# IONIQ6000/av1-go

Hardware: AMD Instinct MI355X
Metric: encoded 4K30 frames/sec (whole node) at fixed QP; PSNR-Y delta vs libaom (higher is better)
Workload: dtype u16

## Files before the change

### av1-go_amd/csrc/av1_entropy_kernels.hip

```cpp
#include <string.h>
#include <vector>
#include "av1_ops_cdfs.hpp"
#include "av1_ops8.hpp"
#include "av1mi_internal.hpp"

namespace av1mi {
using namespace av1ops;

struct Av1EntLaunch {
  FrameView fv;
  int nframes, sbr_n, sbc_n;
  BlockInfo *info;
  op_t *ops; uint32_t ops_cap;
  uint32_t *grouped; uint32_t grouped_cap;
  uint16_t *slot_total, *slot_base;
  uint16_t *rec;
  uint32_t *nops;
  uint8_t *slots; uint32_t slot_cap;
  uint32_t *tile_size;
  uint64_t *tile_off;
  uint32_t *status;
  uint8_t *out; uint64_t out_cap;
  const uint16_t *cdf_image; int cdf_words;
  SlotTable tab;
// ... 4 lines not shown

template <int kKey = -1> __device__ __forceinline__ FrameView frame_view(const Av1EntLaunch &L, int f) {
  FrameView v = L.fv;
  const long nb = (long)v.w8 * v.h8;
  if (kKey < 0 ? v.key != 0 : kKey != 0) { v.y_mode += nb * f; v.uv_mode += nb * f; }
  else { v.mv += nb * 2 * f; v.skip += nb * f; }
  v.lev_y += nb * 64 * f; v.lev_u += nb * 16 * f; v.lev_v += nb * 16 * f;
  v.info = L.info + nb * f;
  if (L.lr_on_frame) for (int p = 0; p < 3; p++) v.lr_on[p] = v.lr_on[p] && L.lr_on_frame[f * 3 + p];
  return v;
}

__global__ __launch_bounds__(256) void k_av1_info(Av1EntLaunch L) {
  const long nb = (long)L.fv.w8 * L.fv.h8, i = (long)blockIdx.x * 256 + threadIdx.x;
  if (i >= nb * L.nframes) return;
  const int f = (int)(i / nb), b = (int)(i - (long)f * nb);
  const FrameView v = frame_view<0>(L, f);
  BlockInfo o = {};
  inter_mode_decision(v, b / v.w8, b % v.w8, &o);
  L.info[nb * f + b] = o;
}

struct TileWave {
  template <class T> using Var = LaneVar<T, 1>;
  template <class F> __device__ __forceinline__ void each(F f) { f((int)threadIdx.x); __syncthreads(); }
  __device__ __forceinline__ int scan(Var<int> &v) {
    const int lane = (int)threadIdx.x, x = v.v[0];
    int inc = x;
#pragma unroll
    for (int d = 1; d < 64; d <<= 1) {
      const int y = __shfl_up(inc, d, 64);
      if (lane >= d) inc += y;
    }
    v.v[0] = inc - x;
    return __shfl(inc, 63, 64);
  }
  __device__ __forceinline__ int first(Var<int> &v) { return __shfl(v.v[0], 0, 64); }
};

__global__ __launch_bounds__(64) __attribute__((amdgpu_waves_per_eu(2, 8))) void k_av1_tokens(Av1EntLaunch L) {
  const int tiles = L.sbr_n * L.sbc_n, t = blockIdx.x, f = t / tiles, tt = t - f * tiles, sbr = tt / L.sbc_n, sbc = tt - sbr * L.sbc_n;
  if (sbr < L.sb_rows32) return;
  const FrameView v = frame_view(L, f);
  __shared__ Tile8Mem S;
  const int below = tiles - L.sb_rows32 * L.sbc_n;
  uint16_t *rec = L.rec + ((size_t)f * below + (tt - (tiles - below))) * kBlocksPerTile * kBlockRecords;
  TileWave w;
  const int n = tok_tile8(w, S, v, sbr, sbc, rec, L.ops + (size_t)t * L.ops_cap, L.ops_cap, L.grouped + (size_t)t * L.grouped_cap,
                          L.slot_total + (size_t)t * S_MAX, L.slot_base + (size_t)t * S_MAX);
  if (threadIdx.x == 0) {
    if (n < 0) atomicOr(L.status, 1u);
    L.nops[t] = n < 0 ? 0u : (uint32_t)n;
  }
}

__global__ __launch_bounds__(64) void k_av1_tokens32(Av1EntLaunch L) {
  __shared__ Tile32Mem S;
  const int tiles = L.sbr_n * L.sbc_n, band = L.sb_rows32 * L.sbc_n, f = blockIdx.x / band, tt = blockIdx.x - f * band, sbr = tt / L.sbc_n, sbc = tt - sbr * L.sbc_n;
  const size_t t = (size_t)f * tiles + tt;
  const FrameView v = frame_view<1>(L, f);
  TileWave w;
  const int n = tok_tile32(w, S, v, sbr, sbc, L.ops + t * L.ops_cap, L.ops_cap, L.grouped + t * L.grouped_cap, L.slot_total + t * S_MAX, L.slot_base + t * S_MAX);
  if (threadIdx.x == 0) {
    if (n < 0) atomicOr(L.status, 1u);
    L.nops[t] = n < 0 ? 0u : (uint32_t)n;
  }
}

__global__ __launch_bounds__(64) void k_av1_chains(Av1EntLaunch L, int ntiles_all, int ngroups) {
  const int xcd = blockIdx.x & 7, j = blockIdx.x >> 3, nslots = L.nslots;
  const int g = (j / nslots) * 8 + xcd, sl = j - (j / nslots) * nslots, lane = threadIdx.x, t = g * 64 + lane;
  if (g >= ngroups) return;
  __shared__ __attribute__((aligned(16))) uint16_t s_big[64 * 16];
  const int n = L.tab.nsym[sl], off = L.tab.off[sl];
  int cnt = 0, base = 0;
  bool mine = t < ntiles_all;
  if (mine && L.band) { const int tiles = L.sbr_n * L.sbc_n, sbr = (t % tiles) / L.sbc_n; mine = (sbr < L.sb_rows32) == (L.band == 1); }
  if (mine) { cnt = L.slot_total[(size_t)t * S_MAX + sl]; base = L.slot_base[(size_t)t * S_MAX + sl]; }
  if (!__any(cnt > 0)) return;
  const size_t tt = t < ntiles_all ? (size_t)t : 0;
  op_t *list = L.ops + tt * L.ops_cap;
  const uint32_t *grouped = L.grouped + tt * L.grouped_cap + base;
  if (n <= 4) {
    const uint32_t *iw = reinterpret_cast<const uint32_t *>(L.cdf_image) + (off >> 1);
    uint64_t cdf = (uint64_t)iw[0] | ((uint64_t)iw[1] << 32);
    const uint4 *g4 = reinterpret_cast<const uint4 *>(grouped);
    const uint4 z = make_uint4(0, 0, 0, 0);
    uint4 c0 = cnt > 0 ? g4[0] : z, c1 = cnt > 4 ? g4[1] : z, c2 = cnt > 8 ? g4[2] : z, c3 = cnt > 12 ? g4[3] : z;
    auto four = [&](const uint4 &v, int e) {
      if (e < cnt) list[v.x >> 4] = small_step(cdf, (int)(v.x & 15), n);
      if (e + 1 < cnt) list[v.y >> 4] = small_step(cdf, (int)(v.y & 15), n);
      if (e + 2 < cnt) list[v.z >> 4] = small_step(cdf, (int)(v.z & 15), n);
      if (e + 3 < cnt) list[v.w >> 4] = small_step(cdf, (int)(v.w & 15), n);
    };
#pragma unroll 1
    for (int e = 0; e < cnt; e += 16) {
      const uint4 *nx = g4 + (e >> 2) + 4;
      const uint4 n0 = e + 16 < cnt ? nx[0] : z, n1 = e + 20 < cnt ? nx[1] : z, n2 = e + 24 < cnt ? nx[2] : z, n3 = e + 28 < cnt ? nx[3] : z;
      four(c0, e); four(c1, e + 4); four(c2, e + 8); four(c3, e + 12);
      c0 = n0; c1 = n1; c2 = n2; c3 = n3;
    }
  } else {
    uint16_t *cdf = s_big + lane * 16;
    {
      const uint4 *iw = reinterpret_cast<const uint4 *>(L.cdf_image + off);
      uint4 *d = reinterpret_cast<uint4 *>(cdf);
      d[0] = iw[0];
      d[1] = n > 8 ? iw[1] : make_uint4(0, 0, 0, 0);
    }
#pragma unroll 1
    for (int e = 0; e < cnt; e++) {
      const uint32_t v = grouped[e];
      const int s = (int)(v & 15);
      list[v >> 4] = s >= kSplitHorz ? split_tuple(cdf, s) : big_step(cdf, s, n);
    }
  }
}

constexpr int kRingOps = 64, kLaneWords = kRingOps * 2 + Coder::kStage + 8;

__global__ __launch_bounds__(64) void k_av1_code(Av1EntLaunch L, int ntiles_all) {
  __shared__ __attribute__((aligned(16))) uint16_t s_lane[64 * kLaneWords];
  const int lane = threadIdx.x, t = blockIdx.x * 64 + lane;
  const bool live = t < ntiles_all;
  uint32_t *ring = reinterpret_cast<uint32_t *>(s_lane + lane * kLaneWords);
  Coder c;
  c.init(L.slots + (size_t)(live ? t : 0) * L.slot_cap, (int)L.slot_cap, s_lane + lane * kLaneWords + kRingOps * 2);
  const int n = live ? (int)L.nops[t] : 0;
  const uint4 *ops4 = reinterpret_cast<const uint4 *>(L.ops + (size_t)(live ? t : 0) * L.ops_cap);
  uint4 r0, r1, r2, r3, r4, r5, r6, r7;
  r0 = r1 = r2 = r3 = r4 = r5 = r6 = r7 = make_uint4(0, 0, 0, 0);
  int w = 0;
  bool pend = false;
  auto request = [&]() {
    const uint4 *p = ops4 + (w >> 2);
    if (w < n) r0 = p[0];
    if (w + 4 < n) r1 = p[1];
    if (w + 8 < n) r2 = p[2];
    if (w + 12 < n) r3 = p[3];
    if (w + 16 < n) r4 = p[4];
    if (w + 20 < n) r5 = p[5];
    if (w + 24 < n) r6 = p[6];
    if (w + 28 < n) r7 = p[7];
    pend = w < n;
  };
  auto take = [&]() {
    uint4 *q = reinterpret_cast<uint4 *>(ring + (w & 32));
    q[0] = r0; q[1] = r1; q[2] = r2; q[3] = r3; q[4] = r4; q[5] = r5; q[6] = r6; q[7] = r7;
    w += 32;
  };
  request();
  if (pend) { take(); request(); }
  int i = 0, lit_left = 0;
  uint32_t op = ring[0], op_next = ring[1], op_next2 = ring[2];
  for (;;) {
    if (!__any(lit_left > 0 || i < n)) break;
    if (__any((pend && w - i < 24) || c.ns >= Coder::kStage - 8)) {
      if (pend && w - i <= 32) { take(); request(); }
      c.spill();
    }
#pragma unroll
    for (int q = 0; q < 8; q++) {
      if (lit_left > 0 || i < n) {
        const uint32_t fetched = ring[(i + 3) & (kRingOps - 1)];
        uint32_t tup = op;
        if (lit_left == 0 && (op >> 31)) lit_left = (int)((op >> 27) & 15);
        if (lit_left > 0) {
          lit_left--;
          tup = (op >> lit_left) & 1 ? (1u << 19) | (256u << 9) : (2u << 19) | (512u << 9) | 256u;
        }
        c.encode_tuple(tup);
        if (lit_left == 0) { i++; op = op_next; op_next = op_next2; op_next2 = fetched; }
      }
    }
  }
  if (!live) return;
  int sz = n ? c.finish() : -1;
  if (sz < 0) { if (n) atomicOr(L.status, 2u); sz = 0; }
  L.tile_size[t] = (uint32_t)sz;
}

__global__ __launch_bounds__(1024) void k_av1_scan(Av1EntLaunch L, int ntiles_all) {
  __shared__ uint64_t part[1024];
  const int tid = threadIdx.x, per = (ntiles_all + 1023) / 1024, i0 = tid * per, i1 = min(i0 + per, ntiles_all);
  uint64_t s = 0;
  for (int i = i0; i < i1; i++) s += L.tile_size[i];
  part[tid] = s;
  __syncthreads();
  for (int d = 1; d < 1024; d <<= 1) {
    const uint64_t y = tid >= d ? part[tid - d] : 0;
    __syncthreads();
    part[tid] += y;
    __syncthreads();
  }
  uint64_t run = part[tid] - s;
  for (int i = i0; i < i1; i++) { L.tile_off[i] = run; run += L.tile_size[i]; }
  if (tid == 1023) {
    L.tile_off[ntiles_all] = part[1023];
    if (part[1023] > L.out_cap) atomicOr(L.status, 4u);
  }
}
__global__ __launch_bounds__(64) void k_av1_gather(Av1EntLaunch L) {
  const int t = blockIdx.x;
  const uint32_t n = L.tile_size[t];
  const uint64_t off = L.tile_off[t];
  if (off + n > L.out_cap) return;
  const uint8_t *src = L.slots + (size_t)t * L.slot_cap;
  uint8_t *dst = L.out + off;
  const uint32_t head = min(n, (uint32_t)((16 - (reinterpret_cast<uintptr_t>(dst) & 15)) & 15)), body = (n - head) >> 4, tail0 = head + (body << 4);
  if (threadIdx.x < head) dst[threadIdx.x] = src[threadIdx.x];
  for (uint32_t i = threadIdx.x; i < body; i += 64) {
    uint4 v;
    __builtin_memcpy(&v, src + head + 16 * i, 16);
    *reinterpret_cast<uint4 *>(dst + head + 16 * i) = v;
  }
  if (tail0 + threadIdx.x < n) dst[tail0 + threadIdx.x] = src[tail0 + threadIdx.x];
}

hipError_t launch_av1_front(av1mi_ctx *ctx, const Av1EntLaunch &L, hipStream_t s) {
  const long nb = (long)L.fv.w8 * L.fv.h8 * L.nframes;
  const int ntiles_all = L.sbr_n * L.sbc_n * L.nframes, ngroups = (ntiles_all + 63) / 64;
  ProfToken t = ctx_prof_begin(ctx, AV1MI_K_ENTROPY_TOKENS, s);
  if (!L.fv.key) hipLaunchKernelGGL(k_av1_info, dim3((unsigned)((nb + 255) / 256)), dim3(256), 0, s, L);
  if (L.sb_rows32 < L.sbr_n) hipLaunchKernelGGL(k_av1_tokens, dim3((unsigned)ntiles_all), dim3(64), 0, s, L);
  if (L.sb_rows32) hipLaunchKernelGGL(k_av1_tokens32, dim3((unsigned)(L.sb_rows32 * L.sbc_n * L.nframes)), dim3(64), 0, s, L);
  ctx_prof_end(ctx, t, s);
  t = ctx_prof_begin(ctx, AV1MI_K_ENTROPY_CHAINS, s);
  Av1EntLaunch C = L;
  C.nslots = L.fv.key ? S_KEY_END : S_INTER_END; C.band = L.sb_rows32 ? 2 : 0;
  if (L.sb_rows32 < L.sbr_n) hipLaunchKernelGGL(k_av1_chains, dim3((unsigned)(((ngroups + 7) / 8) * 8 * C.nslots)), dim3(64), 0, s, C, ntiles_all, ngroups);
  if (L.sb_rows32) {
    C.nslots = K_END; C.band = 1; C.tab = L.tab32; C.cdf_image = L.cdf_image32;
    hipLaunchKernelGGL(k_av1_chains, dim3((unsigned)(((ngroups + 7) / 8) * 8 * C.nslots)), dim3(64), 0, s, C, ntiles_all, ngroups);
  }
  ctx_prof_end(ctx, t, s);
  return hipGetLastError();
}
hipError_t launch_av1_back(av1mi_ctx *ctx, const Av1EntLaunch &L, hipStream_t s) {
  const int ntiles_all = L.sbr_n * L.sbc_n * L.nframes;
  ProfToken t = ctx_prof_begin(ctx, AV1MI_K_ENTROPY, s);
  hipLaunchKernelGGL(k_av1_code, dim3((unsigned)((ntiles_all + 63) / 64)), dim3(64), 0, s, L, ntiles_all);
  ctx_prof_end(ctx, t, s);
  t = ctx_prof_begin(ctx, AV1MI_K_ENTROPY_PACK, s);
  hipLaunchKernelGGL(k_av1_scan, dim3(1), dim3(1024), 0, s, L, ntiles_all);
  hipLaunchKernelGGL(k_av1_gather, dim3((unsigned)ntiles_all), dim3(64), 0, s, L);
  ctx_prof_end(ctx, t, s);
  return hipGetLastError();
}

}

struct av1mi_av1ent_state {
  void *info = nullptr, *ops[2] = { nullptr, nullptr }, *nops[2] = { nullptr, nullptr }, *grouped = nullptr, *slot_tb = nullptr, *rec = nullptr, *slots = nullptr, *tile_off = nullptr, *status = nullptr;
  size_t info_b = 0, ops_b[2] = { 0, 0 }, nops_b[2] = { 0, 0 }, grouped_b = 0, slot_tb_b = 0, rec_b = 0, slots_b = 0, off_b = 0;
  hipEvent_t lists_ready[2] = { nullptr, nullptr }, lists_free[2] = { nullptr, nullptr };
  bool free_recorded[2] = { false, false };
  unsigned long jobs = 0;
  av1mi::Av1EntLaunch pending[2];
  uint64_t *pending_total[2] = { nullptr, nullptr };
  bool pending_valid[2] = { false, false };
  size_t last_tiles = 0;
  uint16_t *d_image[2][4] = {};
  uint16_t *d_image32[4] = {};
  av1ops::SlotTable tab32;
  int image_words[2] = { 0, 0 };
  av1ops::SlotTable tab[2];
};

namespace {
int grow(av1mi_ctx *ctx, void **p, size_t *have, size_t need) {
  if (*have >= need) return AV1MI_OK;
  if (*p) (void)hipFree(*p);
  *p = nullptr; *have = 0;
  if (hipMalloc(p, need) != hipSuccess) return av1mi::ctx_fail(ctx, AV1MI_E_NOMEM, "AV1 entropy scratch: hipMalloc(%zu) failed", need);
  *have = need;
  return AV1MI_OK;
}
}

extern "C" {

uint32_t av1mi_av1_entropy_ops_per_tile(void) { return 32768; }
uint32_t av1mi_av1_entropy_slot_bytes(void) { return 16384; }

}

int av1mi::av1_entropy_front(av1mi_ctx *ctx, const av1mi_av1_entropy_job *j, hipStream_t front, int *ticket) {
  if (!ctx || !ticket) return AV1MI_E_INVAL;
  *ticket = -1;
  if (!j) return av1mi::ctx_fail(ctx, AV1MI_E_INVAL, "null job");
  if (hipSetDevice(av1mi::ctx_device(ctx)) != hipSuccess) return av1mi::ctx_fail(ctx, AV1MI_E_DEVICE, "hipSetDevice failed");
  if (j->width <= 0 || j->height <= 0 || (j->width & 7) || (j->height & 7) || j->width > 4096 || j->height > 4096)
    return av1mi::ctx_fail(ctx, AV1MI_E_INVAL, "frame %dx%d must be a multiple of 8, at most 4096x4096", j->width, j->height);
  if (j->nframes < 0 || j->nframes > 4096 || j->base_q_idx < 1 || j->base_q_idx > 255) return av1mi::ctx_fail(ctx, AV1MI_E_INVAL, "bad nframes / base_q_idx");
  const void *need[] = { j->d_lev_y, j->d_lev_u, j->d_lev_v, j->d_out, j->d_tile_size, j->d_total, j->key ? (const void *)j->d_modes_y : (const void *)j->d_mvs,
                         j->key ? (const void *)j->d_modes_uv : (const void *)j->d_skip };
  for (const void *p : need) if (!p) return av1mi::ctx_fail(ctx, AV1MI_E_INVAL, "null device pointer");
  if (j->nframes == 0) return AV1MI_OK;
  av1mi_av1ent_state *st = av1mi::ctx_av1ent(ctx);
  if (!st) return av1mi::ctx_fail(ctx, AV1MI_E_NOMEM, "AV1 entropy state");
  const int key = j->key ? 1 : 0, qcat = av1ops::q_category(j->base_q_idx);
  if (!st->d_image[key][qcat]) {
    av1ops::SlotTable tab;
    const std::vector<uint16_t> img = av1ops::default_slot_image(key != 0, qcat, &tab);
    st->tab[key] = tab; st->image_words[key] = tab.words;
    if (hipMalloc((void **)&st->d_image[key][qcat], img.size() * 2) != hipSuccess ||
        hipMemcpy(st->d_image[key][qcat], img.data(), img.size() * 2, hipMemcpyHostToDevice) != hipSuccess)
      return av1mi::ctx_fail(ctx, AV1MI_E_DEVICE, "uploading the default CDF image failed");
  }
  if (j->key_rows32 && (!key || (j->key_rows32 & 63) || j->key_rows32 > j->height || (j->width & 31)))
    return av1mi::ctx_fail(ctx, AV1MI_E_INVAL, "key_rows32 %d: whole superblock rows of a key frame whose width is a multiple of 32", j->key_rows32);
  if (j->key_rows32 && !st->d_image32[qcat]) {
    const std::vector<uint16_t> img = av1ops::default_slot_image_k32(qcat, &st->tab32);
    if (hipMalloc((void **)&st->d_image32[qcat], img.size() * 2) != hipSuccess ||
        hipMemcpy(st->d_image32[qcat], img.data(), img.size() * 2, hipMemcpyHostToDevice) != hipSuccess)
      return av1mi::ctx_fail(ctx, AV1MI_E_DEVICE, "uploading the default CDF image failed");
  }
  av1mi::Av1EntLaunch L;
  memset(&L, 0, sizeof(L));
  L.sb_rows32 = j->key_rows32 / 64;
  if (j->key_rows32) { L.tab32 = st->tab32; L.cdf_image32 = st->d_image32[qcat]; }
  L.fv.w8 = j->width / 8; L.fv.h8 = j->height / 8; L.fv.key = key;
  L.fv.y_mode = j->d_modes_y; L.fv.uv_mode = j->d_modes_uv; L.fv.mv = j->d_mvs; L.fv.skip = j->d_skip;
  L.fv.lev_y = j->d_lev_y; L.fv.lev_u = j->d_lev_u; L.fv.lev_v = j->d_lev_v;
  for (int p = 0; p < 3; p++) {
    L.fv.lr_on[p] = j->lr_on[p] != 0;
    const int vh = j->visible_height ? j->visible_height : j->height, vw = j->visible_width ? j->visible_width : j->width;
// ... 94 lines not shown
```

### av1-go_amd/csrc/av1_ops.hpp

```cpp
#pragma once
#include <stdint.h>

#if defined(__HIPCC__)
#include <hip/hip_runtime.h>
#define AV1_HD __host__ __device__ inline
#define AV1_UNROLL _Pragma("unroll")
#define AV1_NOUNROLL _Pragma("unroll 1")
#else
#define AV1_HD inline
#define AV1_UNROLL
#define AV1_NOUNROLL
#endif

namespace av1ops {

typedef uint16_t __attribute__((may_alias)) u16a;
typedef uint32_t __attribute__((may_alias)) u32a;
typedef uint64_t __attribute__((may_alias)) u64a;

enum Slot : int {
  S_SKIP = 0,
  S_PART8 = S_SKIP + 3,
  S_PART16 = S_PART8 + 1,
  S_PART32 = S_PART16 + 4,
// ... 356 lines not shown
    if (c == eob - 1) {
      k.sym(base_eob + (c == 0 ? 0 : c <= nc / 8 ? 1 : c <= nc / 4 ? 2 : 3), imin(a, 3) - 1);
    } else {
      const int mm = imin(m1, 3) + imin(mb, 3) + imin(md, 3) + imin(m2, 3) + imin(mbb, 3);
      int bctx = imin((mm + 1) >> 1, 4);
      if (pos == 0) bctx = 0;
      else bctx += row + col < 2 ? 1 : row + col < 4 ? 6 : 21;
      k.sym(base + bctx, imin(a, 3));
    }
    if (a > 2) {
      int mm = m1 + mb + md;
      mm = imin((mm + 1) >> 1, 6);
      const int rctx = pos == 0 ? mm : (row < 2 && col < 2) ? mm + 7 : mm + 14;
      int rem = a - 3;
      for (int i = 0; i < 4; i++) {
        const int q = imin(rem, 3);
        k.sym(br + rctx, q);
        rem -= q;
        if (q < 3) break;
      }
    }
  }
}
template <int N, const BandSlots &B, class K, class M_>
AV1_HD void tok_coeffs_pass2(K &k, const M_ &M, bool chroma, const int16_t *lev, int above_dc, int left_dc, int c_lo, int c_hi) {
  const int LG = M.LG, MS = M.MS;
  for (int c = c_lo; c < c_hi; c++) {
    const int pos = M.pos(c), m = M.at((pos >> LG) * MS + (pos & (N - 1)));
    if (!m) continue;
    const int neg = M.neg(pos);
    if (c == 0) {
      const int sg = (above_dc == 2) - (above_dc == 1) + (left_dc == 2) - (left_dc == 1);
      k.sym((chroma ? B.dc_sign_c : B.dc_sign_y) + (sg < 0 ? 1 : sg > 0 ? 2 : 0), neg);
    } else {
      k.lit((unsigned)neg, 1);
    }
    if (m == 15) {
      const int a = iabs(lev[pos]);
      if (a > 14) {
        const unsigned x = (unsigned)(a - 14);
        const int len = ilog2(x) + 1;
        k.lit(0, len - 1);
        k.lit(x, len);
      }
    }
  }
}
template <int N, const BandSlots &B, class K, class TS>
AV1_HD void tok_coeffs(K &k, const TS &ts, bool chroma, const int16_t *lev, int above_cul, int above_dc, int left_cul, int left_dc, int tx_slot,
                       int tx_sym) {
  MagMap<N> M(ts);
  const int eob = M.load(lev);
  tok_coeffs_lead<N, B>(k, chroma, eob, above_cul, above_dc, left_cul, left_dc, tx_slot, tx_sym);
  if (!eob) return;
  tok_coeffs_pass1<N, B>(k, M, chroma, lev, eob, eob - 1, 0);
  tok_coeffs_pass2<N, B>(k, M, chroma, lev, above_dc, left_dc, 0, eob);
}

AV1_HD void tok_mv_comp(Sink &k, int comp, int diff) {
  const int base = S_MV_COMP + comp * 16;
  k.sym(base + MVC_SIGN, diff < 0);
  const int off = iabs(diff) - 1, cls = (off >> 3) < 2 ? 0 : ilog2((unsigned)(off >> 3));
  k.sym(base + MVC_CLASS, cls);
  if (cls == 0) {
    k.sym(base + MVC_CLASS0, off >> 3);
    k.sym(base + MVC_CLASS0_FR + (off >> 3), (off >> 1) & 3);
  } else {
    const int o = off - (2 << (cls + 2)), d = o >> 3;
    for (int i = 0; i < cls; i++) k.sym(base + MVC_BITS + i, (d >> i) & 1);
    k.sym(base + MVC_FR, (o >> 1) & 3);
  }
}

AV1_HD void tok_block(const FrameView &f, Sink &k, const TokScratch &ts, int sbr, int sbc, int zi, const uint8_t *sums) {
  int bx, by;
  demorton8((unsigned)zi, &bx, &by);
  const int r8 = sbr * 8 + by, c8 = sbc * 8 + bx;
  if (r8 >= f.h8 || c8 >= f.w8) return;
  if (zi == 0) tok_lr<kSlots8>(f, k, sbr, sbc);
  tok_partition_prefix(f, k, sbr, sbc, bx, by);
  const int b = r8 * f.w8 + c8;
  const bool au = by > 0, al = bx > 0;
  const unsigned sa = au ? sums[(by - 1) * 8 + bx] : 0u, sl = al ? sums[by * 8 + bx - 1] : 0u;
  const int skip = f.key ? 0 : f.skip[b];
  k.sym(S_SKIP + (au && !f.key ? f.skip[b - f.w8] : 0) + (al && !f.key ? f.skip[b - 1] : 0), skip);
  int ym = 0;
  if (f.key) {
    ym = f.y_mode[b];
    tok_kf_modes<kSlots8>(k, ym, f.uv_mode[b], au ? f.y_mode[b - f.w8] : 0, al ? f.y_mode[b - 1] : 0);
  } else {
    k.sym(S_IS_INTER + 0, 1);
    const int rctx = (au || al) ? 1 : 0;
    k.sym(S_SINGLE_REF + rctx * 3 + 0, 0);
    k.sym(S_SINGLE_REF + rctx * 3 + 1, 0);
    k.sym(S_SINGLE_REF + rctx * 3 + 2, 0);
    const BlockInfo me = f.info[b];
    const int mode = me.mode & 3, ref_idx = me.mode >> 2, num = me.num;
    const int mx = f.mv[2 * b], my = f.mv[2 * b + 1];
    const int close = (au ? 1 : 0) + (al ? 1 : 0);
    int num_new = (au ? f.info[b - f.w8].flags & 1 : 0) + (al ? f.info[b - 1].flags & 1 : 0);
    if (au && bx < 7 && c8 + 1 < f.w8 && morton8((unsigned)bx + 1, (unsigned)by - 1) < morton8((unsigned)bx, (unsigned)by)) num_new += f.info[b - f.w8 + 1].flags & 1;
    const int new_ctx = close == 0 ? 0 : close == 1 ? 3 - imin(num_new, 1) : 5 - imin(num_new, 1);
    const int ref_ctx = close == 0 ? 0 : close == 1 ? 3 : 5;
    k.sym(S_NEW_MV + new_ctx, mode != 3);
    if (mode != 3) {
      k.sym(S_ZERO_MV, mode != 2);
      if (mode != 2) k.sym(S_REF_MV + ref_ctx, mode == 1);
    }
    auto drl_ctx = [&](int i) {
      const bool a = (me.drl >> i) & 1, c = (me.drl >> (i + 1)) & 1;
      return a && c ? 0 : a ? 1 : !c ? 2 : 0;
    };
    if (mode == 3) {
      for (int i = 0; i < 2; i++)
        if (num > i + 1) {
          k.sym(S_DRL + drl_ctx(i), ref_idx != i);
          if (ref_idx == i) break;
        }
      const int dx = mx - me.px, dy = my - me.py;
      k.sym(S_MV_JOINT, (dx ? 1 : 0) + (dy ? 2 : 0));
      if (dy) tok_mv_comp(k, 0, dy);
      if (dx) tok_mv_comp(k, 1, dx);
    } else if (mode == 1) {
      for (int i = 1; i < 3; i++)
        if (num > i + 1) {
          k.sym(S_DRL + drl_ctx(i), ref_idx != i);
          if (ref_idx == i) break;
        }
    }
  }
  if (skip) return;
  tok_coeffs<8, kSlots8>(k, ts, false, f.lev_y + (long)b * 64, 0, summary_dc(sa, 0), 0, summary_dc(sl, 0), f.key ? S_INTRA_TX + ym : S_INTER_TX, f.key ? 1 : 7);
  AV1_NOUNROLL
  for (int p = 1; p < 3; p++)
    tok_coeffs<4, kSlots8>(k, ts, true, (p == 1 ? f.lev_u : f.lev_v) + (long)b * 16, summary_cul(sa, p), summary_dc(sa, p), summary_cul(sl, p), summary_dc(sl, p), -1, 0);
}

template <class F> AV1_HD void build_slot_table(int n, F nsym, SlotTable *t) {
  int o = 0;
  for (int s = 0; s < S_MAX; s++) {
    if (s < n) {
      t->nsym[s] = (uint8_t)nsym(s);
      const int w = slot_words(t->nsym[s]), al = w < 8 ? 4 : 8;
      o = (o + al - 1) & ~(al - 1);
      t->off[s] = (uint16_t)o;
      o += w;
    } else { t->nsym[s] = 2; t->off[s] = 0; }
  }
  t->words = (o + 7) & ~7;
}
AV1_HD void build_slot_table(bool key, SlotTable *t) { build_slot_table(key ? S_KEY_END : S_INTER_END, [key](int s) { return slot_nsym(s, key); }, t); }

#ifdef AV1_CODER_STATS
static long long coder_stat_carries = 0;
#endif
struct Coder {
  enum { kStage = 32 };
  uint64_t low;
  uint32_t rng;
  int nb;
  uint8_t *out;
  uint16_t *stage;
  int pos, cap, ns;
  bool overflow;
  AV1_HD void init(uint8_t *o, int c, uint16_t *st) { low = 0; rng = 0x8000; nb = -1; out = o; stage = st; pos = 0; cap = c; ns = 0; overflow = false; }
  AV1_HD void carry_back() {
    for (int k = ns; k-- > 0;) { const uint16_t v = (uint16_t)(stage[k] + 1); stage[k] = v; if (v) return; }
    for (int i = pos; i-- > 0;) if (++out[i] != 0) return;
  }
  AV1_HD bool stage_full() const { return ns >= kStage - 1; }
  AV1_HD void spill() {
    if (pos + 2 * ns > cap) { overflow = true; pos += 2 * ns; ns = 0; return; }
    for (int k = 0; k < ns; k++) { const uint32_t v = stage[k]; *reinterpret_cast<uint16_t *>(out + pos + 2 * k) = (uint16_t)((v >> 8) | (v << 8)); }
    pos += 2 * ns; ns = 0;
  }
  AV1_HD void flush16() {
    nb -= 16;
    const uint32_t w = (uint32_t)(low >> (16 + nb));
    if ((w >> 16) && !overflow) {
#ifdef AV1_CODER_STATS
      coder_stat_carries++;
#endif
      carry_back();
    }
    stage[ns++] = (uint16_t)w;
    low &= ((uint64_t)1 << (16 + nb)) - 1;
  }
  AV1_HD void encode(uint32_t fl, uint32_t fh, int s, int n) {
    const uint32_t r = rng, v = (((r >> 8) * (fh >> 6)) >> 1) + 4u * (uint32_t)(n - 1 - s);
    const uint32_t u = fl < 32768u ? (((r >> 8) * (fl >> 6)) >> 1) + 4u * (uint32_t)(n - s) : r;
    low += r - u;
    const uint32_t nr = u - v;
    const int d = 15 - ilog2(nr);
    rng = nr << d; low <<= d; nb += d;
    if (nb >= 32) flush16();
  }
  AV1_HD void encode_tuple(op_t t) {
    const uint32_t fl6 = (t >> 9) & 1023u, fh6 = t & 511u, dl = (t >> 19) & 31u;
    const uint32_t r = rng, v = (((r >> 8) * fh6) >> 1) + 4u * (dl - 1u);
    const uint32_t u = fl6 < 512u ? (((r >> 8) * fl6) >> 1) + 4u * dl : r;
    low += r - u;
    const uint32_t nr = u - v;
    const int d = 15 - ilog2(nr);
    rng = nr << d; low <<= d; nb += d;
    if (nb >= 32) flush16();
  }
  AV1_HD void bit(int b) { encode(b ? 16384u : 32768u, b ? 0u : 16384u, b, 2); }
  AV1_HD int finish() {
    uint64_t e = ((low + 0x3FFF) & ~(uint64_t)0x3FFF) | 0x4000;
    if (nb >= 0 && (e >> (16 + nb))) { if (!overflow) carry_back(); e &= ((uint64_t)1 << (16 + nb)) - 1; }
    spill();
    int top = 15 + nb;
    while (top >= 14) {
      uint8_t byte = 0;
      for (int q = 7; q >= 0 && top >= 14; q--, top--) byte |= (uint8_t)(((e >> top) & 1) << q);
      if (pos < cap) out[pos] = byte; else overflow = true;
      pos++;
    }
    return overflow ? -1 : pos;
  }
};

AV1_HD uint32_t adapt(uint32_t x, bool below, int rate) {
  const uint32_t m = 0u - (uint32_t)below, d = ((x ^ m) + (m & 32769u)) >> rate;
  return x - ((d ^ m) - m);
}

AV1_HD op_t small_step(uint64_t &w, int s, int n) {
  const uint32_t x0 = (uint32_t)w & 0xFFFFu, x1 = (uint32_t)w >> 16, x2 = (uint32_t)(w >> 32) & 0xFFFFu, cnt = (uint32_t)(w >> 48);
  const uint32_t fl = s == 0 ? 32768u : s == 1 ? x0 : s == 2 ? x1 : x2;
  const uint32_t fh = s == n - 1 ? 0u : s == 0 ? x0 : s == 1 ? x1 : x2;
  const int rate = 3 + (cnt > 15) + (cnt > 31) + (n >= 4 ? 2 : 1);
  const uint32_t y0 = adapt(x0, 0 < s, rate), y1 = adapt(x1, 1 < s, rate), y2 = adapt(x2, 2 < s, rate), ncnt = cnt + (cnt < 32);
  w = (uint64_t)(y0 | (y1 << 16)) | ((uint64_t)(y2 | (ncnt << 16)) << 32);
  return make_tuple(fl, fh, s, n);
}

AV1_HD op_t big_step(uint16_t *v, int s, int n) {
  const int nd = n > 8 ? 8 : 4;
  u32a *d = reinterpret_cast<u32a *>(v);
  uint32_t w[8];
  AV1_UNROLL
  for (int k = 0; k < 8; k++) w[k] = k < nd ? d[k] : 0u;
  const uint32_t fl = s ? v[s - 1] : 32768u, fh = s == n - 1 ? 0u : v[s];
  const uint32_t cnt = (nd == 8 ? w[7] : w[3]) >> 16;
  const int rate = 3 + (cnt > 15) + (cnt > 31) + 2;
  AV1_UNROLL
  for (int k = 0; k < 8; k++) {
    if (k >= nd) continue;
    uint32_t lo = adapt(w[k] & 0xFFFFu, 2 * k < s, rate), hi = adapt(w[k] >> 16, 2 * k + 1 < s, rate);
    if (k == nd - 1) hi = cnt + (cnt < 32);
    d[k] = lo | (hi << 16);
  }
  return make_tuple(fl, fh, s, n);
}

AV1_HD op_t split_tuple(const uint16_t *p, int kind) {
  const uint32_t p1 = p[0] - p[1], p2 = p[1] - p[2], p3 = p[2] - p[3], p4 = p[3] - p[4], p5 = p[4] - p[5], p6 = p[5] - p[6], p7 = p[6] - p[7],
                 p8 = p[7] - p[8], p9 = p[8];
  return make_tuple(kind == kSplitHorz ? p2 + p3 + p4 + p6 + p7 + p9 : p1 + p3 + p4 + p5 + p6 + p8, 0, 1, 2);
}

AV1_HD void run_chain(const uint16_t *init, int n, const uint32_t *g, int cnt, op_t *list) {
  if (n <= 4) {
    uint64_t w = (uint64_t)init[0] | ((uint64_t)init[1] << 16) | ((uint64_t)init[2] << 32) | ((uint64_t)init[3] << 48);
    for (int k = 0; k < cnt; k++) list[g[k] >> 4] = small_step(w, (int)(g[k] & 15), n);
    return;
  }
  alignas(16) uint16_t v[16];
  for (int i = 0; i < 16; i++) v[i] = i < slot_words(n) ? init[i] : 0;
  for (int k = 0; k < cnt; k++) {
    const int s = (int)(g[k] & 15);
    list[g[k] >> 4] = s >= kSplitHorz ? split_tuple(v, s) : big_step(v, s, n);
  }
}

AV1_HD void code_word(Coder &c, op_t e) {
  if (e >> 31) { for (int i = (int)((e >> 27) & 15) - 1; i >= 0; i--) { c.bit((e >> i) & 1); if (c.stage_full()) c.spill(); } }
  else { c.encode_tuple(e); if (c.stage_full()) c.spill(); }
}

}
```

### av1-go_amd/host/av1_opstream.cpp

```cpp
#include <algorithm>
#include <cstdio>
#include <cstdlib>
#include <cstring>
#include <string>
#include <vector>
#include "../csrc/av1_ops_cdfs.hpp"
#include "../csrc/av1_ops8.hpp"
#include "av1_bitstream.hpp"

namespace av1mi_host {
namespace av1 {

bool opstream_supported(const av1mi_obu_frame &f, std::string *why) {
  auto no = [&](const char *m) { if (why) *why = m; return false; };
  if (f.cdef_bits || f.reduced_tx_set || f.disable_cdf_update) return no("cdef_bits / reduced_tx_set / disable_cdf_update must be 0");
  if (f.tile_cols_log2 >= 0 || f.tile_rows_log2 >= 0) return no("one superblock per tile only");
  if (f.angle_y || f.angle_uv || f.cfl_alpha || f.tx_type || f.is_inter) return no("angle deltas, chroma from luma, transform types and intra blocks in inter frames are host-writer only");
  if (f.frame_type == 0 && f.skip) return no("key frames are coded with skip = 0");
  for (int p = 0; p < 3; p++) if (f.lr_type[p] > 1) return no("Wiener restoration only");
  if (f.lr_unit_shift || f.lr_uv_shift) return no("64x64 restoration units only");
  return true;
}

namespace {
bool code_list(std::vector<av1ops::op_t> &list, const std::vector<uint32_t> &grouped, int nslots, const uint16_t *total, const uint16_t *base,
               const av1ops::SlotTable &tab, const uint16_t *image, std::vector<uint8_t> *out, std::string *err) {
  using namespace av1ops;
  const int nops = (int)list.size();
  for (int sl = 0; sl < nslots; sl++)
    if (total[sl]) run_chain(&image[tab.off[sl]], tab.nsym[sl], &grouped[(size_t)base[sl]], total[sl], list.data());
  out->resize((size_t)nops * 2 + 64);
  Coder c;
  uint16_t stage[Coder::kStage];
  c.init(out->data(), (int)out->size(), stage);
  for (int i = 0; i < nops; i++) code_word(c, list[(size_t)i]);
  const int n = c.finish();
  if (n < 0) { if (err) *err = "tile payload overflow"; return false; }
  out->resize((size_t)n);
  return true;
}
struct WaveLoop {
  template <class T> using Var = av1ops::LaneVar<T, av1ops::kLanes32>;
  template <class F> void each(F f) { for (int lane = 0; lane < av1ops::kLanes32; lane++) f(lane); }
  int scan(Var<int> &v) {
    int run = 0;
    for (int lane = 0; lane < av1ops::kLanes32; lane++) { const int x = v.v[lane]; v.v[lane] = run; run += x; }
    return run;
  }
  int first(Var<int> &v) { return v.v[0]; }
};
void frame_view_of(const av1mi_obu_frame &f, av1ops::FrameView *v) {
  memset(v, 0, sizeof(*v));
  v->w8 = f.width / 8; v->h8 = f.height / 8; v->key = f.frame_type == 0;
  v->y_mode = f.y_mode; v->uv_mode = f.uv_mode; v->mv = f.mv; v->skip = f.skip; v->lev_y = f.lev_y; v->lev_u = f.lev_u; v->lev_v = f.lev_v;
  for (int p = 0; p < 3; p++) {
    v->lr_on[p] = f.lr_type[p] == 1;
    const int ph = p ? (visible_height(f) + 1) >> 1 : visible_height(f), pw = p ? (visible_width(f) + 1) >> 1 : visible_width(f);
    v->lr_rows[p] = std::max((ph + 32) / 64, 1); v->lr_cols[p] = std::max((pw + 32) / 64, 1);
  }
}
bool lr_units_of(const av1mi_obu_frame &f, av1ops::FrameView *v, std::string *err) {
  for (int p = 0; p < 3; p++) {
    if (!v->lr_on[p]) continue;
    const int8_t *u = f.lr_units[p];
    const size_t n = (size_t)v->lr_rows[p] * v->lr_cols[p];
    for (size_t i = 1; i < n; i++) if (memcmp(u, u + i * 8, 8)) { if (err) *err = "restoration units must be uniform per plane"; return false; }
    if (p == 2 && v->lr_on[1] && memcmp(u, f.lr_units[1], 8)) { if (err) *err = "U and V restoration units must be equal"; return false; }
    memcpy(v->lr_unit[p ? 1 : 0], u, 8);
  }
  return true;
}
}

bool opstream_tiles(const av1mi_obu_frame &f, std::vector<std::vector<uint8_t>> *tiles, std::string *err, int key_rows32) {
  using namespace av1ops;
  if (!opstream_supported(f, err)) return false;
  if (key_rows32 && (f.frame_type != 0 || (key_rows32 & 63) || key_rows32 > f.height || (f.width & 31))) { if (err) *err = "bad 32x32 band"; return false; }
  FrameView v;
  frame_view_of(f, &v);
  std::vector<uint8_t> zskip;
  if (!v.key && !v.skip) { zskip.assign((size_t)v.w8 * v.h8, 0); v.skip = zskip.data(); }
  if (!lr_units_of(f, &v, err)) return false;
  const size_t nb = (size_t)v.w8 * v.h8;
  std::vector<BlockInfo> info(nb);
  v.info = info.data();
  for (size_t b = 0; b < nb; b++) memset(&info[b], 0, sizeof(BlockInfo));
  if (!v.key) for (int r = 0; r < v.h8; r++) for (int c = 0; c < v.w8; c++) inter_mode_decision(v, r, c, &info[(size_t)r * v.w8 + c]);
  const int qcat = q_category(f.base_q_idx);
  SlotTable tab;
  const std::vector<uint16_t> image = default_slot_image(v.key != 0, qcat, &tab);
  const int sbr_n = (v.h8 + 7) / 8, sbc_n = (v.w8 + 7) / 8;
  tiles->assign((size_t)sbr_n * sbc_n, {});
  const int nslots = v.key ? S_KEY_END : S_INTER_END;
  std::vector<Tile8Mem> mem8(1);
  std::vector<uint16_t> rec((size_t)kBlocksPerTile * kBlockRecords);
  const uint32_t ops_cap8 = 1u << 20;
  std::vector<op_t> list8(ops_cap8);
  std::vector<uint32_t> grouped8(65536 + kListAlign);
  const bool stats = getenv("AV1MI_TOK_STATS") != nullptr;
  int st_rec = 0, st_cnt = 0, st_ops = 0, st_over = 0; long st_ops_sum = 0;
  SlotTable tab32;
  const std::vector<uint16_t> image32 = key_rows32 ? default_slot_image_k32(qcat, &tab32) : std::vector<uint16_t>();
  std::vector<Tile32Mem> mem32(key_rows32 ? 1 : 0);
  const uint32_t ops_cap32 = 1u << 20;
  std::vector<op_t> list32(key_rows32 ? ops_cap32 : 0);
  std::vector<uint32_t> grouped32(key_rows32 ? 65536 : 0);
  for (int sbr = 0; sbr < sbr_n; sbr++)
    for (int sbc = 0; sbc < sbc_n; sbc++) {
      if (sbr * 64 < key_rows32) {
        WaveLoop wave;
        uint16_t base[S_MAX], total[S_MAX];
        const int words = tok_tile32(wave, mem32[0], v, sbr, sbc, list32.data(), ops_cap32, grouped32.data(), total, base);
        if (words < 0) { if (err) *err = "tile too large for 16-bit entry positions"; return false; }
        std::vector<op_t> list(list32.begin(), list32.begin() + words);
        if (!code_list(list, grouped32, K_END, total, base, tab32, image32.data(), &(*tiles)[(size_t)sbr * sbc_n + sbc], err)) return false;
        continue;
      }
      WaveLoop wave;
      uint16_t base[S_MAX], total[S_MAX];
      const int words = tok_tile8(wave, mem8[0], v, sbr, sbc, rec.data(), list8.data(), ops_cap8, grouped8.data(), total, base);
      if (stats) {
        std::vector<uint8_t> cnt((size_t)S_MAX * kBlocksPerTile, 0);
        const TokScratch ts = { mem8[0].p1.mag, &mem8[0].scan };
        int ops = 0;
        for (int zi = 0; zi < kBlocksPerTile; zi++) {
          Sink k = { rec.data(), cnt.data(), zi, 0, 0, false };
          tok_block(v, k, ts, sbr, sbc, zi, mem8[0].sums);
          st_rec = std::max(st_rec, k.nrec); ops += k.n;
        }
        for (uint8_t c : cnt) st_cnt = std::max(st_cnt, (int)c);
        st_ops = std::max(st_ops, ops); st_ops_sum += ops;
        if (words < 0) { st_over++; continue; }
      }
      if (words < 0) { if (err) *err = "a tile exceeds the tokenizer's capacities (records or symbols of a slot per block, entries per tile)"; return false; }
      std::vector<op_t> list(list8.begin(), list8.begin() + words);
      if (!code_list(list, grouped8, nslots, total, base, tab, image.data(), &(*tiles)[(size_t)sbr * sbc_n + sbc], err)) return false;
    }
  if (stats)
    fprintf(stderr, "[av1mi tok stats] %d tiles: records per block <= %d (capacity %d), symbols of a slot in a block <= %d (255), list words per tile <= %d, mean %.0f; %d tiles over a block capacity\n",
            sbr_n * sbc_n, st_rec, (int)kBlockRecords, st_cnt, st_ops, (double)st_ops_sum / (sbr_n * sbc_n), st_over);
  return true;
}

int opstream_slots() { return av1ops::S_MAX; }

int opstream_tile8(const av1mi_obu_frame &f, int sbr, int sbc, uint32_t ops_cap, uint32_t *list, uint32_t *grouped, uint16_t *slot_total, uint16_t *slot_base,
                   std::string *err) {
  using namespace av1ops;
  if (!opstream_supported(f, err) || sbr < 0 || sbc < 0 || sbr * 64 >= f.height || sbc * 64 >= f.width) return -2;
  FrameView v;
  frame_view_of(f, &v);
  std::vector<uint8_t> zskip;
  if (!v.key && !v.skip) { zskip.assign((size_t)v.w8 * v.h8, 0); v.skip = zskip.data(); }
  if (!lr_units_of(f, &v, err)) return -2;
  std::vector<BlockInfo> info(v.key ? 0 : (size_t)v.w8 * v.h8);
  v.info = info.data();
  if (!v.key) for (int r = 0; r < v.h8; r++) for (int c = 0; c < v.w8; c++) { memset(&info[(size_t)r * v.w8 + c], 0, sizeof(BlockInfo)); inter_mode_decision(v, r, c, &info[(size_t)r * v.w8 + c]); }
  std::vector<Tile8Mem> mem(1);
  std::vector<uint16_t> rec((size_t)kBlocksPerTile * kBlockRecords);
  WaveLoop wave;
  return tok_tile8(wave, mem[0], v, sbr, sbc, rec.data(), list, ops_cap, grouped, slot_total, slot_base);
}

int opstream_tile32(const av1mi_obu_frame &f, int sbr, int sbc, uint32_t ops_cap, uint32_t *list, uint32_t *grouped, uint16_t *slot_total, uint16_t *slot_base,
                    std::string *err) {
  using namespace av1ops;
  if (!opstream_supported(f, err) || f.frame_type != 0 || (f.width & 31) || sbr < 0 || sbc < 0 || (sbr + 1) * 64 > f.height || sbc * 64 >= f.width) return -2;
  FrameView v;
  frame_view_of(f, &v);
  if (!lr_units_of(f, &v, err)) return -2;
  std::vector<Tile32Mem> mem(1);
  WaveLoop wave;
  return tok_tile32(wave, mem[0], v, sbr, sbc, list, ops_cap, grouped, slot_total, slot_base);
}

}
}
```

### av1-go_amd/host/coder_selftest.cpp

```cpp
#include <stdint.h>
#include <string.h>
#include <vector>
#include "av1_bitstream.hpp"
#define AV1_CODER_STATS
namespace coder_selftest {
#include "../csrc/av1_ops.hpp"
}

extern "C" long long av1mi_host_coder_selftest(uint64_t seed, long long count, long long *carries) {
  using coder_selftest::av1ops::Coder;
  std::vector<uint32_t> fl((size_t)count), fh((size_t)count);
  std::vector<uint8_t> sy((size_t)count), ns((size_t)count);
  uint64_t x = seed * 0x9E3779B97F4A7C15ull + 1;
  auto rnd = [&]() { x ^= x << 13; x ^= x >> 7; x ^= x << 17; return (uint32_t)(x >> 16); };
  for (long long i = 0; i < count; i++) {
    const int n = 2 + (int)(rnd() % 15);
    int s;
    uint32_t a, b;
    s = (int)(rnd() % (uint32_t)n);
    const uint32_t hi = 32768u - 64u * (uint32_t)s, lo = 64u * (uint32_t)(n - 1 - s);
    a = s == 0 ? 32768u : lo + 64u + rnd() % (hi - lo - 63u);
    b = s == n - 1 ? 0u : lo + rnd() % (a - 63u - lo);
    fl[(size_t)i] = a; fh[(size_t)i] = b; sy[(size_t)i] = (uint8_t)s; ns[(size_t)i] = (uint8_t)n;
  }
  const std::vector<uint8_t> ref = av1mi_host::av1::range_code_raw(fl.data(), fh.data(), sy.data(), ns.data(), (size_t)count);
  std::vector<uint8_t> out((size_t)count * 2 + 64);
  coder_selftest::av1ops::coder_stat_carries = 0;
  Coder c;
  uint16_t stage[Coder::kStage];
  c.init(out.data(), (int)out.size(), stage);
  for (long long i = 0; i < count; i++) {
    c.encode(fl[(size_t)i], fh[(size_t)i], sy[(size_t)i], ns[(size_t)i]);
    if (c.stage_full()) c.spill();
  }
  const int sz = c.finish();
  if (carries) *carries = coder_selftest::av1ops::coder_stat_carries;
  if (sz < 0 || (size_t)sz != ref.size()) return -1;
  for (size_t i = 0; i < ref.size(); i++) if (out[i] != ref[i]) return (long long)i + 1;
  return 0;
}
```

Before: 2941.

## Make range coder branchless with deferred carries and add fast 8-op path

The coder's renormalisation is rewritten as a branchless update that always writes a staged word and records carries in a bitmask, resolving them only at spill time instead of walking backwards on each carry. The GPU tile-coding loop gains a fast path: when no lane in the wavefront has a long literal in its next eight ops, all eight are encoded without per-op literal bookkeeping, using a prefetched window. This targets branch divergence and serial dependencies in the per-lane entropy coder. It adds register pressure and extra unconditional stage writes, and a host code_ops path and step tests are added to check bit-exactness.

```diff
diff --git a/av1-go_amd/csrc/av1_entropy_kernels.hip b/av1-go_amd/csrc/av1_entropy_kernels.hip
--- a/av1-go_amd/csrc/av1_entropy_kernels.hip
+++ b/av1-go_amd/csrc/av1_entropy_kernels.hip
@@ -180,13 +180,42 @@
   request();
   if (pend) { take(); request(); }
   int i = 0, lit_left = 0;
-  uint32_t op = ring[0], op_next = ring[1], op_next2 = ring[2];
+  uint32_t x[8];
+  auto window = [&](int from) {
+#pragma unroll
+    for (int j = 0; j < 8; j++) if (j >= from) x[j] = ring[(i + j) & (kRingOps - 1)];
+  };
+  window(0);
   for (;;) {
-    if (!__any(lit_left > 0 || i < n)) break;
+    const int rem = n - i;
+    if (!__any(lit_left > 0 || rem > 0)) break;
     if (__any((pend && w - i < 24) || c.ns >= Coder::kStage - 8)) {
       if (pend && w - i <= 32) { take(); request(); }
       c.spill();
     }
+    uint32_t m = 0;
+    if (__any(rem > 0 && rem < 8)) {
+#pragma unroll
+      for (int j = 0; j < 8; j++) m = max(m, j < rem ? x[j] : 0u);
+    } else {
+      m = max(max(max(x[0], x[1]), max(x[2], x[3])), max(max(x[4], x[5]), max(x[6], x[7])));
+      m = rem > 0 ? m : 0u;
+    }
+    if (!__any(lit_left > 0 || m >= kLongLiteral)) {
+      uint32_t y[8];
+#pragma unroll
+      for (int j = 0; j < 8; j++) y[j] = ring[(i + 8 + j) & (kRingOps - 1)];
+#pragma unroll
+      for (int q = 0; q < 8; q++) {
+        const uint32_t tup = (int)x[q] < 0 ? bit_tuple(x[q] & 1u) : x[q];
+        c.encode_tuple(q < rem ? tup : kNullTuple);
+      }
+      i += min(max(rem, 0), 8);
+#pragma unroll
+      for (int j = 0; j < 8; j++) x[j] = y[j];
+      continue;
+    }
+    uint32_t op = x[0], op_next = x[1], op_next2 = x[2];
 #pragma unroll
     for (int q = 0; q < 8; q++) {
       if (lit_left > 0 || i < n) {
@@ -195,12 +224,14 @@
         if (lit_left == 0 && (op >> 31)) lit_left = (int)((op >> 27) & 15);
         if (lit_left > 0) {
           lit_left--;
-          tup = (op >> lit_left) & 1 ? (1u << 19) | (256u << 9) : (2u << 19) | (512u << 9) | 256u;
+          tup = bit_tuple((op >> lit_left) & 1u);
         }
         c.encode_tuple(tup);
         if (lit_left == 0) { i++; op = op_next; op_next = op_next2; op_next2 = fetched; }
       }
     }
+    x[0] = op; x[1] = op_next; x[2] = op_next2;
+    window(3);
   }
   if (!live) return;
   int sz = n ? c.finish() : -1;
diff --git a/av1-go_amd/csrc/av1_ops.hpp b/av1-go_amd/csrc/av1_ops.hpp
--- a/av1-go_amd/csrc/av1_ops.hpp
+++ b/av1-go_amd/csrc/av1_ops.hpp
@@ -532,63 +532,73 @@
 AV1_HD void build_slot_table(bool key, SlotTable *t) { build_slot_table(key ? S_KEY_END : S_INTER_END, [key](int s) { return slot_nsym(s, key); }, t); }
 
 #ifdef AV1_CODER_STATS
-static long long coder_stat_carries = 0;
+static long long coder_stat_carries = 0, coder_stat_wrapped = 0, coder_stat_stored = 0;
 #endif
 struct Coder {
   enum { kStage = 32 };
   uint64_t low;
   uint32_t rng;
   int nb;
+  uint32_t carry_mask;
   uint8_t *out;
   uint16_t *stage;
   int pos, cap, ns;
   bool overflow;
-  AV1_HD void init(uint8_t *o, int c, uint16_t *st) { low = 0; rng = 0x8000; nb = -1; out = o; stage = st; pos = 0; cap = c; ns = 0; overflow = false; }
-  AV1_HD void carry_back() {
-    for (int k = ns; k-- > 0;) { const uint16_t v = (uint16_t)(stage[k] + 1); stage[k] = v; if (v) return; }
+  AV1_HD void init(uint8_t *o, int c, uint16_t *st) { low = 0; rng = 0x8000; nb = -1; carry_mask = 0; out = o; stage = st; pos = 0; cap = c; ns = 0; overflow = false; }
+  AV1_HD void carry_back(int k) {
+#ifdef AV1_CODER_STATS
+    coder_stat_carries++;
+    if (k > 0 && stage[k - 1] == 0xFFFFu) coder_stat_wrapped++;
+#endif
+    while (k-- > 0) { const uint16_t v = (uint16_t)(stage[k] + 1); stage[k] = v; if (v) return; }
+#ifdef AV1_CODER_STATS
+    if (pos > 0) coder_stat_stored++;
+#endif
     for (int i = pos; i-- > 0;) if (++out[i] != 0) return;
+  }
+  AV1_HD void resolve() {
+    while (carry_mask) {
+      const int k = ilog2(carry_mask);
+      carry_mask ^= 1u << k;
+      if (!overflow) carry_back(k);
+    }
   }
   AV1_HD bool stage_full() const { return ns >= kStage - 1; }
   AV1_HD void spill() {
+    resolve();
     if (pos + 2 * ns > cap) { overflow = true; pos += 2 * ns; ns = 0; return; }
     for (int k = 0; k < ns; k++) { const uint32_t v = stage[k]; *reinterpret_cast<uint16_t *>(out + pos + 2 * k) = (uint16_t)((v >> 8) | (v << 8)); }
     pos += 2 * ns; ns = 0;
   }
-  AV1_HD void flush16() {
-    nb -= 16;
-    const uint32_t w = (uint32_t)(low >> (16 + nb));
-    if ((w >> 16) && !overflow) {
-#ifdef AV1_CODER_STATS
-      coder_stat_carries++;
-#endif
-      carry_back();
-    }
-    stage[ns++] = (uint16_t)w;
-    low &= ((uint64_t)1 << (16 + nb)) - 1;
+  AV1_HD void update(uint32_t a, uint32_t nr) {
+    const int d = __builtin_clz(nr) - 16;
+    rng = nr << d;
+    low = (low + a) << d;
+    const int k = nb + d - 32;
+    const bool f = k >= 0;
+    const uint32_t kk = (uint32_t)k < 31u ? (uint32_t)k : 31u, hi = (uint32_t)(low >> 32);
+    const uint32_t w = hi >> kk;
+    low = (uint64_t)(uint32_t)low | ((uint64_t)(hi & ((1u << kk) - 1u)) << 32);
+    stage[ns] = (uint16_t)w;
+    carry_mask |= (w >> 16) << ns;
+    ns += f;
+    nb = f ? k + 16 : k + 32;
   }
   AV1_HD void encode(uint32_t fl, uint32_t fh, int s, int n) {
     const uint32_t r = rng, v = (((r >> 8) * (fh >> 6)) >> 1) + 4u * (uint32_t)(n - 1 - s);
     const uint32_t u = fl < 32768u ? (((r >> 8) * (fl >> 6)) >> 1) + 4u * (uint32_t)(n - s) : r;
-    low += r - u;
-    const uint32_t nr = u - v;
-    const int d = 15 - ilog2(nr);
-    rng = nr << d; low <<= d; nb += d;
-    if (nb >= 32) flush16();
+    update(r - u, u - v);
   }
   AV1_HD void encode_tuple(op_t t) {
     const uint32_t fl6 = (t >> 9) & 1023u, fh6 = t & 511u, dl = (t >> 19) & 31u;
     const uint32_t r = rng, v = (((r >> 8) * fh6) >> 1) + 4u * (dl - 1u);
     const uint32_t u = fl6 < 512u ? (((r >> 8) * fl6) >> 1) + 4u * dl : r;
-    low += r - u;
-    const uint32_t nr = u - v;
-    const int d = 15 - ilog2(nr);
-    rng = nr << d; low <<= d; nb += d;
-    if (nb >= 32) flush16();
+    update(r - u, u - v);
   }
   AV1_HD void bit(int b) { encode(b ? 16384u : 32768u, b ? 0u : 16384u, b, 2); }
   AV1_HD int finish() {
     uint64_t e = ((low + 0x3FFF) & ~(uint64_t)0x3FFF) | 0x4000;
-    if (nb >= 0 && (e >> (16 + nb))) { if (!overflow) carry_back(); e &= ((uint64_t)1 << (16 + nb)) - 1; }
+    if (nb >= 0 && (e >> (16 + nb))) { carry_mask |= 1u << ns; e &= ((uint64_t)1 << (16 + nb)) - 1; }
     spill();
     int top = 15 + nb;
     while (top >= 14) {
@@ -660,4 +670,23 @@
   else { c.encode_tuple(e); if (c.stage_full()) c.spill(); }
 }
 
-}
+constexpr op_t kLongLiteral = 0x90000000u, kNullTuple = (1u << 19) | (512u << 9);
+AV1_HD op_t bit_tuple(uint32_t b) { return b ? (1u << 19) | (256u << 9) : (2u << 19) | (512u << 9) | 256u; }
+
+AV1_HD void code_ops(Coder &c, const op_t *list, int n) {
+  int i = 0, lit_left = 0;
+  while (lit_left > 0 || i < n) {
+    if (c.ns >= Coder::kStage - 8) c.spill();
+    for (int q = 0; q < 8; q++) {
+      if (!(lit_left > 0 || i < n)) break;
+      const op_t op = list[i];
+      op_t tup = op;
+      if (lit_left == 0 && (op >> 31)) lit_left = (int)((op >> 27) & 15);
+      if (lit_left > 0) { lit_left--; tup = bit_tuple((op >> lit_left) & 1); }
+      c.encode_tuple(tup);
+      if (lit_left == 0) i++;
+    }
+  }
+}
+
+}
diff --git a/av1-go_amd/host/av1_opstream.cpp b/av1-go_amd/host/av1_opstream.cpp
--- a/av1-go_amd/host/av1_opstream.cpp
+++ b/av1-go_amd/host/av1_opstream.cpp
@@ -33,7 +33,7 @@
   Coder c;
   uint16_t stage[Coder::kStage];
   c.init(out->data(), (int)out->size(), stage);
-  for (int i = 0; i < nops; i++) code_word(c, list[(size_t)i]);
+  code_ops(c, list.data(), nops);
   const int n = c.finish();
   if (n < 0) { if (err) *err = "tile payload overflow"; return false; }
   out->resize((size_t)n);
diff --git a/av1-go_amd/host/coder_selftest.cpp b/av1-go_amd/host/coder_selftest.cpp
--- a/av1-go_amd/host/coder_selftest.cpp
+++ b/av1-go_amd/host/coder_selftest.cpp
@@ -39,3 +39,72 @@
   for (size_t i = 0; i < ref.size(); i++) if (out[i] != ref[i]) return (long long)i + 1;
   return 0;
 }
+
+extern "C" long long av1mi_host_coder_steptest(uint64_t seed, long long count, int mode, long long *stats) {
+  using namespace coder_selftest::av1ops;
+  std::vector<uint32_t> fl, fh;
+  std::vector<uint8_t> sy, ns;
+  std::vector<op_t> list;
+  uint64_t x = seed * 0x9E3779B97F4A7C15ull + 1;
+  auto rnd = [&]() { x ^= x << 13; x ^= x >> 7; x ^= x << 17; return (uint32_t)(x >> 16); };
+  uint32_t r = 0x8000, diff = rnd() % 0x8000u;
+  long long follow = 0;
+  auto new_run = [&]() { const uint32_t k = rnd() % 8; follow = k < 3 ? 18 + rnd() % 24 : k < 6 ? 40 + rnd() % 400 : 600 + rnd() % 1200; };
+  new_run();
+  auto choose = [&](int n, const uint32_t *icdf) {
+    int s = (int)(rnd() % (uint32_t)n);
+    auto uv = [&](int t, uint32_t *u, uint32_t *v) {
+      const uint32_t a = t ? icdf[t - 1] : 32768u, b = t == n - 1 ? 0u : icdf[t];
+      *v = (((r >> 8) * (b >> 6)) >> 1) + 4u * (uint32_t)(n - 1 - t);
+      *u = a < 32768u ? (((r >> 8) * (a >> 6)) >> 1) + 4u * (uint32_t)(n - t) : r;
+    };
+    uint32_t u, v;
+    bool crossed = false;
+    if (mode == 1) {
+      for (s = 0; s < n; s++) { uv(s, &u, &v); if (diff < r - v) break; }
+      if (follow <= 0 && s < n - 1) { s++; crossed = true; }
+    }
+    uv(s, &u, &v);
+    const uint32_t nr = u - v;
+    const int d = __builtin_clz(nr) - 16;
+    diff = crossed ? rnd() % nr << d : (diff - (r - u)) << d;
+    r = nr << d;
+    follow -= d;
+    if (crossed) new_run();
+    fl.push_back(s ? icdf[s - 1] : 32768u); fh.push_back(s == n - 1 ? 0u : icdf[s]); sy.push_back((uint8_t)s); ns.push_back((uint8_t)n);
+    return s;
+  };
+  for (long long i = 0; i < count; i++) {
+    const bool literal = mode >= 2 || rnd() % 4 == 0;
+    if (literal) {
+      const int k = mode == 2 ? 1 : mode == 3 ? 11 : 1 + (int)(rnd() % 11);
+      const uint32_t half = 16384u;
+      unsigned val = 0;
+      for (int b = 0; b < k; b++) val = (val << 1) | (unsigned)choose(2, &half);
+      list.push_back(op_lit(k, val));
+    } else {
+      const int n = 2 + (int)(rnd() % 15);
+      uint32_t icdf[16];
+      uint32_t top = 511;
+      for (int j = 0; j < n - 1; j++) { const uint32_t room = top - (uint32_t)(n - 1 - j); icdf[j] = 64u * ((uint32_t)(n - 1 - j) + rnd() % room); top = icdf[j] / 64u; }
+      const int s = choose(n, icdf);
+      list.push_back(make_tuple(fl.back(), fh.back(), s, n));
+    }
+  }
+  const std::vector<uint8_t> ref = av1mi_host::av1::range_code_raw(fl.data(), fh.data(), sy.data(), ns.data(), sy.size());
+  std::vector<uint8_t> out(sy.size() * 2 + 64), out2(out.size());
+  uint16_t stage[Coder::kStage];
+  Coder c;
+  c.init(out2.data(), (int)out2.size(), stage);
+  for (op_t e : list) code_word(c, e);
+  const int sz2 = c.finish();
+  coder_stat_carries = coder_stat_wrapped = coder_stat_stored = 0;
+  c.init(out.data(), (int)out.size(), stage);
+  code_ops(c, list.data(), (int)list.size());
+  const int sz = c.finish();
+  if (stats) { stats[0] = coder_stat_carries; stats[1] = coder_stat_wrapped; stats[2] = coder_stat_stored; stats[3] = (long long)list.size(); }
+  if (sz < 0 || (size_t)sz != ref.size()) return -1;
+  for (size_t i = 0; i < ref.size(); i++) if (out[i] != ref[i]) return (long long)i + 1;
+  if (sz2 != sz || memcmp(out.data(), out2.data(), (size_t)sz)) return 1ll << 40;
+  return 0;
+}
diff --git a/av1-go_amd/host/coder_steptest_main.cpp b/av1-go_amd/host/coder_steptest_main.cpp
--- /dev/null
+++ b/av1-go_amd/host/coder_steptest_main.cpp
@@ -0,0 +1,23 @@
+#include <stdint.h>
+#include <stdio.h>
+extern "C" long long av1mi_host_coder_selftest(uint64_t seed, long long count, long long *carries);
+extern "C" long long av1mi_host_coder_steptest(uint64_t seed, long long count, int mode, long long *stats);
+
+int main() {
+  int bad = 0;
+  long long st[4];
+  for (uint64_t seed = 0; seed < 4; seed++) {
+    bad += av1mi_host_coder_steptest(seed, 300000, 0, st) != 0;
+    bad += av1mi_host_coder_steptest(seed, 200000, 1, st) != 0;
+    printf("seed %d: %lld carries, %lld through 0xFFFF entries, %lld into stored bytes\n", (int)seed, st[0], st[1], st[2]);
+  }
+  const long long counts[] = { 1, 7, 8, 9, 40000 };
+  for (long long n : counts) bad += av1mi_host_coder_steptest(5, n, 2, st) != 0;
+  bad += av1mi_host_coder_steptest(5, 1, 3, st) != 0;
+  bad += av1mi_host_coder_steptest(5, 3, 3, st) != 0;
+  bad += av1mi_host_coder_steptest(5, 40000, 3, st) != 0;
+  for (long long n = 0; n <= 40; n++) for (int mode = 0; mode < 2; mode++) bad += av1mi_host_coder_steptest((uint64_t)n + 11, n, mode, st) != 0;
+  bad += av1mi_host_coder_selftest(1, 2000000, st) != 0;
+  printf("%s\n", bad ? "FAILED" : "OK");
+  return bad != 0;
+}
```

Measured after the change: 2975, median of 6. +1.2%, better.
